# 1879615351/Go-RIO

Hardware: AMD Instinct MI355X
Metric: APD-GICP GN iters/sec on 16k-pt scans + GP-preint windows/sec (higher is better)
Workload: dtype f32 search / f64 accumulate; 1 GPU; C4: 64 scan pairs 16384x16384 + 64 GP windows 1 s @ 200 Hz per GPU, k-NN covariances + 20 fixed GN iterations per pair; pairs_per_gpu=64, target_points=16384, optimizer=GN (convergence test disabled), search=pruned, parallelism=batch shard x1 (no collective)

## Files before the change

go-rio_amd/csrc/ugpm_api.hip:

```cpp
#include <hip/hip_runtime.h>

#include <algorithm>
#include <cstdlib>
#include <chrono>
#include <cstdio>
#include <cstring>
#include <limits>
#include <memory>
#include <string>
#include <atomic>
#include <vector>

#include "../../include/gorio_ugpm.h"
#include "dev_buffer.h"
#include "ugpm_kernels.hip"
#include "ugpm_lpm_out.hip"
#include "ugpm_chunks.h"
#include "ugpm_windows.h"

using namespace gorio;
using namespace gorio::windows;

namespace {

// ... 58 lines not shown
  PinnedBuf pin_out;
  DevBuf<double> lpm_ws;
  DevBuf<int> lpm_ints;
  DevBuf<ug::LpmOutWin> d_lpm_wins;
  struct StageEvents { hipEvent_t a, b; int stage; };
  std::vector<StageEvents> ev;

  void drop_stage_events() {
    for (auto& e : ev) { hipEventDestroy(e.a); hipEventDestroy(e.b); }
    ev.clear();
  }
  void reset() {
    if (device >= 0) hipSetDevice(device);
    for (size_t g = 1; g < groups.size(); ++g) destroy_stream_pair(groups[g]);
    for (Group& g : groups) { hipEventDestroy(g.ev_done); hipEventDestroy(g.ev_tab); }
    groups.clear();
    destroy_stream_pair(main);
    if (ev_up) hipEventDestroy(ev_up);
    ev_up = nullptr;
    drop_stage_events();
    ws.reset(); d_wins.reset(); d_ints.reset(); d_diag.reset(); pin_in.reset(); pin_out.reset(); lpm_ws.reset(); lpm_ints.reset(); d_lpm_wins.reset();
    wins_cap = 0;
    lm_budget[0] = lm_budget[1] = 0;
    device = -1;
  }
  ~Ctx() { reset(); }
};
thread_local Ctx g_ctx;

struct Stage {
  Ctx& c;
  hipStream_t stream;
  size_t slot = 0;
  bool on = false;
  Stage(Ctx& c_, int s, hipStream_t st = nullptr) : c(c_), stream(st ? st : c_.main.s) {
    hipEvent_t a = nullptr, b = nullptr;
    if (hipEventCreate(&a) != hipSuccess || hipEventCreate(&b) != hipSuccess) return;
    slot = c.ev.size();
    c.ev.push_back({a, b, s});
    hipEventRecord(a, stream);
    on = true;
  }
  ~Stage() {
    if (on) hipEventRecord(c.ev[slot].b, stream);
  }
};
struct StageEventsGuard {
  Ctx& c;
  ~StageEventsGuard() { c.drop_stage_events(); }
};

struct Run : Ctx::Group {
  int g0 = 0, nw = 0;
  const UgpmWin* wins = nullptr;
  bool active = true;
};

struct Batch {
  const gorio_ugpm_window* windows;
  int nw;
  std::vector<HostWin> hw;
  std::vector<UgpmWin> dw;
  std::vector<int> ints, flags, lpm_ints_h;
  std::vector<double> lpm_in;
  std::vector<ug::LpmOutWin> lw;
  std::vector<size_t> out_offs;
  std::vector<Run> runs;
  size_t total_doubles = 0, total_in = 0, total_out = 0;
  double* out_region = nullptr;
  int max_S = 0, max_G = 2, max_V = 2, max_infer = 0, n_lpm = 0;
  bool rerun = false;
  bool looks = false;
  bool enqueued_blind[2] = {false, false};
  std::vector<int> final_status;
  int first_error = 0;
  std::string first_error_msg;
  void note_error(int i, int code, const std::string& m) {
    if (first_error) return;
    first_error = code;
    first_error_msg = "window " + std::to_string(i) + ": " + m;
  }
};

int ensure_context(Ctx& c, int device) {
  int ndev = 0;
  if (hipGetDeviceCount(&ndev) != hipSuccess || ndev <= 0) return ufail(GORIO_UGPM_ERR_NO_DEVICE, "no usable HIP device (no CPU fallback exists)");
  if (device < 0 || device >= ndev) return ufail(GORIO_UGPM_ERR_INVALID, "bad device ordinal");
  if (c.device != device) c.reset();
  UHIP(hipSetDevice(device));
  if (c.device == device) return 0;
  if (int rc = make_stream_pair(c.main)) return rc;
  UHIP(hipFuncSetAttribute(reinterpret_cast<const void*>(&ug::corr_diag_kernel<kSolveKmaxSmall>), hipFuncAttributeMaxDynamicSharedMemorySize, 140 * 1024));
  UHIP(hipFuncSetAttribute(reinterpret_cast<const void*>(&ug::corr_diag_kernel<kSolveKmaxFull>), hipFuncAttributeMaxDynamicSharedMemorySize, 140 * 1024));
  UHIP(hipFuncSetAttribute(reinterpret_cast<const void*>(&ug::infer_kernel<kSolveKmaxSmall>), hipFuncAttributeMaxDynamicSharedMemorySize, 17 * (6 * 160 + 16) * 8));
  UHIP(hipFuncSetAttribute(reinterpret_cast<const void*>(&ug::infer_kernel<kSolveKmaxFull>), hipFuncAttributeMaxDynamicSharedMemorySize, 17 * (6 * 160 + 16) * 8) );
  const void* fns[] = {reinterpret_cast<const void*>(&ug::ata_kernel<4, 16, kAtaTilesCorr>), reinterpret_cast<const void*>(&ug::ata_kernel<8, 16, kAtaTilesCorr>),
                       reinterpret_cast<const void*>(&ug::ata_kernel<16, 8, kAtaTilesCorr>), reinterpret_cast<const void*>(&ug::ata_kernel<4, 16, kAtaTilesLm>),
                       reinterpret_cast<const void*>(&ug::ata_kernel<8, 16, kAtaTilesLm>)};
  for (const void* f : fns) UHIP(hipFuncSetAttribute(f, hipFuncAttributeMaxDynamicSharedMemorySize, 144 * 1024));
  c.device = device;
  return 0;
}

void plan_windows(Batch& b) {
  b.hw.resize(b.nw);
  int total_infer = 0;
  for (int i = 0; i < b.nw; ++i) {
    const gorio_ugpm_window& w = b.windows[i];
    HostWin& h = b.hw[i];
    total_infer += std::max(0, w.n_infer);
    b.max_infer = std::max(b.max_infer, w.n_infer);
    std::string err;
    if (plan_window(w, h, err) != 0) {
      b.note_error(i, h.status, err);
    } else if (h.is_lpm) {
      b.n_lpm++;
    } else {
      b.max_S = std::max(b.max_S, h.S);
      b.total_in += input_slot(w, h);
      b.total_doubles += h.ws_doubles;
    }
  }
  for (const HostWin& h : b.hw) {
    b.max_G = std::max(b.max_G, h.is_lpm ? 2 : h.G);
    b.max_V = std::max(b.max_V, h.is_lpm ? 2 : h.V);
  }
  b.total_out = (size_t)total_infer * 83;
  b.total_doubles += b.total_in + b.total_out + 64;
}

int reserve_workspace(Ctx& c, const Batch& b) {
  const size_t nw = b.nw;
  UHIP(c.ws.reserve(b.total_doubles));
  UHIP(reserve_group(c.wins_cap, nw, nw, c.d_wins, nw, c.d_ints, kWinInts * nw, c.d_diag, 4 * nw));
  UHIP(c.pin_in.reserve(sizeof(double) * b.total_in, sizeof(double) * (b.total_in + b.total_in / 4 + 64)));
  const size_t down = sizeof(double) * (b.total_out + 4 * nw) + sizeof(int) * kWinInts * nw;
  UHIP(c.pin_out.reserve(down, down + down / 4 + 64));
  return 0;
}

int stage_and_upload(Ctx& c, Batch& b) {
  b.dw.resize(b.nw);
  b.ints.assign(kWinInts * (size_t)b.nw, 0);
  b.out_offs.assign(b.nw, 0);
  double* const in_region = c.ws.get();
  b.out_region = in_region + b.total_in;
  double* base = b.out_region + (b.total_out + 31) / 32 * 32;
  double* const stage_in = static_cast<double*>(c.pin_in.get());
  size_t in_off = 0, out_off = 0;
  for (int i = 0; i < b.nw; ++i) {
    const gorio_ugpm_window& w = b.windows[i];
    const HostWin& h = b.hw[i];
    UgpmWin& u = b.dw[i];
    std::memset(&u, 0, sizeof(u));
    u.lmi = c.d_ints + kWinInts * (size_t)i;
    u.status = c.d_ints + kWinInts * (size_t)i + 16;
    b.ints[kWinInts * (size_t)i + 16] = h.status;
    u.n_infer = std::max(0, w.n_infer);
    b.out_offs[i] = out_off;
    u.out = b.out_region + out_off;
    out_off += (size_t)u.n_infer * 83;
    if (h.status != 0) continue;
    if (h.is_lpm) {
      b.ints[kWinInts * (size_t)i + 16] = 1;
      u.n_infer = 0;
      continue;
    }
    carve(w, h, u, base, in_region + in_off, u.out);
    u.G = h.G; u.V = h.V; u.S = h.S;
    u.correlate = w.correlate ? 1 : 0; u.overlap = w.overlap;
    u.state_freq = h.state_freq;
    copy_noise_and_priors(w, u);
    base += h.ws_doubles;
    double* s = stage_in + in_off;
    const size_t padded = input_slot(w, h);
    for (size_t k = padded - 4; k < padded; ++k) s[k] = 0.0;
    s = stage_samples(s, w, h.g0, h.G, h.v0, h.V);
    std::copy(h.state_t.begin(), h.state_t.end(), s);
    in_off += padded;
  }
  if (b.total_in) UHIP(hipMemcpyAsync(in_region, stage_in, sizeof(double) * b.total_in, hipMemcpyHostToDevice, c.main.s));
  UHIP(hipMemcpyAsync(c.d_wins, b.dw.data(), sizeof(UgpmWin) * b.nw, hipMemcpyHostToDevice, c.main.s));
// ... 13 lines not shown
    LpmHost& L = lh[widx.size()];
    build_lpm_timeline(b.windows[i], L);
    widx.push_back(i);
    max_T = std::max(max_T, (int)L.tl.size());
    ug::LpmOutWin dummy;
    const LpmSize sz = carve_lpm(b.windows[i], L.tl.size(), dummy, nullptr, nullptr, nullptr);
    in_dbl += sz.in;
    dbl += sz.scratch + 8;
    nint += sz.ints;
  }
  UHIP(c.lpm_ws.reserve(in_dbl + dbl));
  UHIP(c.lpm_ints.reserve(nint));
  UHIP(c.d_lpm_wins.reserve(b.n_lpm));
  b.lw.resize(widx.size());
  b.lpm_in.assign(in_dbl, 0.0);
  b.lpm_ints_h.assign(nint, 0);
  LpmSize at;
  for (size_t k = 0; k < widx.size(); ++k) {
    const int i = widx[k];
    const gorio_ugpm_window& w = b.windows[i];
    const LpmHost& L = lh[k];
    ug::LpmOutWin& u = b.lw[k];
    std::memset(&u, 0, sizeof(u));
    const LpmSize sz = carve_lpm(w, L.tl.size(), u, c.lpm_ws.get() + at.in, c.lpm_ws.get() + in_dbl + at.scratch, c.lpm_ints.get() + at.ints);
    std::copy(L.tl.begin(), L.tl.end(), stage_samples(b.lpm_in.data() + at.in, w, 0, w.n_gyr, 0, w.n_vel));
    stage_lpm_tables(b.lpm_ints_h.data() + at.ints, L);
    at.in += sz.in; at.scratch += sz.scratch; at.ints += sz.ints;
    u.G = w.n_gyr; u.V = w.n_vel; u.T = (int)L.tl.size(); u.n_infer = w.n_infer;
    u.start_index = L.start_index; u.dt_index = L.dt_index;
    copy_noise_and_priors(w, u);
    u.out = b.dw[i].out;
    u.status = c.d_ints + kWinInts * (size_t)i + 17;
  }
  UHIP(hipMemcpyAsync(c.lpm_ws, b.lpm_in.data(), sizeof(double) * in_dbl, hipMemcpyHostToDevice, c.main.s));
  UHIP(hipMemcpyAsync(c.lpm_ints, b.lpm_ints_h.data(), sizeof(int) * nint, hipMemcpyHostToDevice, c.main.s));
  UHIP(hipMemcpyAsync(c.d_lpm_wins, b.lw.data(), sizeof(ug::LpmOutWin) * b.lw.size(), hipMemcpyHostToDevice, c.main.s));
  const int nl = (int)b.lw.size();
  if (nl > 0) {
    Stage st(c, 0);
    ug::lpm_out_steps_kernel<<<dim3((max_T + 255) / 256, 5, nl), 256, 0, c.main.s>>>(c.d_lpm_wins);
    ug::lpm_out_scan_kernel<<<dim3(5, nl), 64, 0, c.main.s>>>(c.d_lpm_wins);
    ug::lpm_out_finish_kernel<<<nl, 256, 0, c.main.s>>>(c.d_lpm_wins);
    UHIP(hipGetLastError());
  }
  return 0;
}

int open_groups(Ctx& c, Batch& b) {
  int n_groups = 1;
  if (const char* e = std::getenv("GORIO_UGPM_GROUPS")) n_groups = std::atoi(e);
  n_groups = std::max(1, std::min(std::min(n_groups, 8), b.nw));
  while ((int)c.groups.size() < n_groups) {
    Ctx::Group g;
    if (c.groups.empty()) static_cast<StreamPair&>(g) = c.main;
    else if (int rc = make_stream_pair(g)) return rc;
    UHIP(hipEventCreateWithFlags(&g.ev_done, hipEventDisableTiming));
    UHIP(hipEventCreateWithFlags(&g.ev_tab, hipEventDisableTiming));
    c.groups.push_back(g);
  }
  if (!c.ev_up) UHIP(hipEventCreateWithFlags(&c.ev_up, hipEventDisableTiming));
  UHIP(hipEventRecord(c.ev_up, c.main.s));
  b.runs.resize(n_groups);
  for (int g = 0; g < n_groups; ++g) {
    Run& r = b.runs[g];
    static_cast<Ctx::Group&>(r) = c.groups[g];
    r.g0 = (int)((long)b.nw * g / n_groups);
    r.nw = (int)((long)b.nw * (g + 1) / n_groups) - r.g0;
    r.wins = c.d_wins + r.g0;
    if (g > 0) UHIP(hipStreamWaitEvent(r.s, c.ev_up, 0));
  }
  return 0;
}

void launch_ata(Ctx& c, int max_S, const Run& r, int which, int decide = 0) {
  hipStream_t sq = which == 2 ? r.s2 : r.s;
  Stage st_ata(c, which == 2 ? 6 : 5, sq);
  const int n = (which == 2 ? 6 : 3) * max_S;
  const int tpg = which == 2 ? kAtaTilesCorr : kAtaTilesLm;
  const int dense = (g_debug_path.load() & 1) ? 1 : 0;
  const int ng = ata_cut(n, which == 2 && !dense ? 3 * max_S : n, tpg).groups();
  const int npad = ((n + 15) / 32) * 32 + 16;
  const int grid = ((r.nw + 7) / 8) * ng * 8;
  auto lds = [&](int kc) { return sizeof(double) * 2 * kc * (npad + 1); };
  if (which == 2) {
    if (npad <= 256) ug::ata_kernel<4, 16, kAtaTilesCorr><<<grid, 512, lds(16), sq>>>(r.wins, which, r.nw, ng, decide, dense);
    else if (npad <= 512) ug::ata_kernel<8, 16, kAtaTilesCorr><<<grid, 512, lds(16), sq>>>(r.wins, which, r.nw, ng, decide, dense);
    else ug::ata_kernel<16, 8, kAtaTilesCorr><<<grid, 512, lds(8), sq>>>(r.wins, which, r.nw, ng, decide, dense);
  } else {
    if (npad <= 256) ug::ata_kernel<4, 16, kAtaTilesLm><<<grid, 512, lds(16), sq>>>(r.wins, which, r.nw, ng, decide, dense);
    else ug::ata_kernel<8, 16, kAtaTilesLm><<<grid, 512, lds(16), sq>>>(r.wins, which, r.nw, ng, decide, dense);
  }
}

SolverSizes batch_sizes(const Batch& b) { return solver_sizes(b.max_S, (g_debug_path.load() & 4) != 0); }

void launch_gram(const Run& r, const SolverSizes& z) {
  const dim3 grid(6, r.nw);
  if (z.gram_rows == kGramRowsSmall) ug::gram_kernel<kGramRowsSmall, kGramKmax><<<grid, 256, 0, r.s>>>(r.wins);
  else if (z.gram_rows == kGramRows) ug::gram_kernel<kGramRows, kGramKmax><<<grid, 256, 0, r.s>>>(r.wins);
  else ug::gram_kernel<kCholRowsFull, kSolveKmaxFull><<<grid, 256, 0, r.s>>>(r.wins);
}

void launch_lm_step(const Run& r, const SolverSizes& z, int problem) {
  const dim3 grid(r.nw, problem == 1 ? kVelBlocks : 1);
  if (z.lm_rows == kLmRowsSmall) ug::lm_step_kernel<kLmRowsSmall><<<grid, 512, 0, r.s>>>(r.wins);
  else ug::lm_step_kernel<kCholRowsFull><<<grid, 512, 0, r.s>>>(r.wins);
}

void launch_corr_diag(const Run& r, const SolverSizes& z, int max_S) {
  const dim3 grid((6 * max_S + 15) / 16, r.nw);
  const size_t lds = sizeof(double) * 17 * (6 * max_S + 16);
  if (z.solve_kmax == kSolveKmaxSmall) ug::corr_diag_kernel<kSolveKmaxSmall><<<grid, 256, lds, r.s2>>>(r.wins);
  else ug::corr_diag_kernel<kSolveKmaxFull><<<grid, 256, lds, r.s2>>>(r.wins);
}

void launch_infer(const Run& r, const SolverSizes& z, int max_S, int max_infer) {
  const dim3 grid(std::max(1, max_infer), r.nw);
  const size_t lds = sizeof(double) * 17 * (6 * max_S + 16);
  if (z.solve_kmax == kSolveKmaxSmall) ug::infer_kernel<kSolveKmaxSmall><<<grid, 256, lds, r.s>>>(r.wins);
  else ug::infer_kernel<kSolveKmaxFull><<<grid, 256, lds, r.s>>>(r.wins);
}

int enqueue_tables_and_correlation(Ctx& c, Batch& b) {
  const int max_S = b.max_S;
  const SolverSizes sizes = batch_sizes(b);
  for (const Run& r : b.runs) {
    {
      Stage st(c, 0, r.s);
      ug::lpm_rot_kernel<<<dim3(r.nw, 5), 320, 0, r.s>>>(r.wins);
      ug::lpm_init_kernel<<<r.nw, 320, 0, r.s>>>(r.wins);
    }
    {
      Stage st(c, 1, r.s);
      launch_gram(r, sizes);
      ug::cross_kernel<<<dim3(12, r.nw, (std::max(b.max_G, b.max_V) + ug::kCrossRows - 1) / ug::kCrossRows), 256, sizeof(double) * ug::kCrossRows * (((max_S + 31) / 32) * 32 + 4), r.s>>>(r.wins);
    }
    UHIP(hipEventRecord(r.ev_tab, r.s));
    UHIP(hipStreamWaitEvent(r.s2, r.ev_tab, 0));
    {
      Stage st(c, 2, r.s2);
      ug::corr_jac_kernel<<<dim3(ug::kCorrJacParts, r.nw), 256, 0, r.s2>>>(r.wins);
      UHIP(hipEventRecord(r.ev_jac, r.s2));
      launch_ata(c, max_S, r, 2);
      ug::corr_factor_kernel<<<r.nw, 512, 0, r.s2>>>(r.wins);
      launch_corr_diag(r, sizes, max_S);
    }
    UHIP(hipEventRecord(r.ev_corr, r.s2));
  }
  return 0;
}

int run_fit(Ctx& c, Batch& b, int problem) {
  const int max_S = b.max_S;
  const SolverSizes sizes = batch_sizes(b);
  std::vector<int>& flags = b.flags;
  const bool lmtrace = std::getenv("GORIO_UGPM_LMTRACE") != nullptr;
  const bool speculative = g_speculative_rot.load() != 0;
  std::vector<std::unique_ptr<Stage>> st_lm;
  for (Run& r : b.runs) {
    st_lm.emplace_back(new Stage(c, 3, r.s));
    if (problem == 0) ug::rot_eval_kernel<<<dim3(r.nw, kEvalSplit), 256, 0, r.s>>>(r.wins, 2);
    else ug::vel_eval_kernel<<<dim3(r.nw, kEvalSplit), 256, 0, r.s>>>(r.wins, 2);
    launch_ata(c, max_S, r, problem);
    r.active = true;
  }
  for (int it = 0; it <= 51; ++it) {
    bool any = false;
    for (Run& r : b.runs) {
      if (!r.active) continue;
      any = true;
      launch_lm_step(r, sizes, problem);
      if (problem == 0 && speculative) {
        ug::rot_eval_kernel<<<dim3(r.nw, kEvalSplit), 256, 0, r.s>>>(r.wins, 3);
        launch_ata(c, max_S, r, problem, 1);
// ... 339 lines not shown
```

go-rio_amd/csrc/ugpm_device.h:

```cpp
#pragma once
#include <stdint.h>

namespace gorio {

constexpr int kAtaTilesLm = 24, kAtaTilesCorr = 48;
constexpr int kWinInts = 48;
constexpr int kLmiNeed = 18;
constexpr int kStatusUnfinished = 2;
constexpr int kCholRowsFull = 384;
constexpr int kVelBlocks = 3;

#if defined(__HIPCC__)
#define GORIO_HD __host__ __device__
#else
#define GORIO_HD
#endif

struct AtaCut {
  int ntile, q_zero, ng_dense, ng_skip;
  GORIO_HD int groups() const { return ng_dense + ng_skip; }
  GORIO_HD bool skips(int grp) const { return grp >= ng_dense; }
  GORIO_HD int q_lo(int grp) const {
    return grp < ng_dense ? (int)((long)grp * q_zero / ng_dense) : q_zero + (int)((long)(grp - ng_dense) * (ntile - q_zero) / ng_skip);
  }
  GORIO_HD int q_hi(int grp) const { return grp + 1 == groups() ? ntile : q_lo(grp + 1); }
};
GORIO_HD inline AtaCut ata_cut(int n, int zero_col, int tpg) {
  const int T = (n + 15) / 16, tz = zero_col >= n ? T : (zero_col + 15) / 16;
  AtaCut c;
  c.ntile = T * (T + 1) / 2;
  c.q_zero = tz * (tz + 1) / 2;
  c.ng_dense = (c.q_zero + tpg - 1) / tpg;
  c.ng_skip = (c.ntile - c.q_zero + tpg - 1) / tpg;
  return c;
}

struct UgpmWin {
  const double* gyr_t;
  const double* gyr;
  const double* vel_t;
  const double* vel;
  const double* infer_t;
  double* state_t;
  int G, V, S, n_infer;
  int correlate, overlap;
  double start_t, state_freq, gyr_var, vel_var;
  double gyr_bias[3], vel_bias[3];
  double vel_bias_std, gyr_bias_std;
  double* Rq;
  double* Rstart;
  double* velr;
  double* dp;
  double* r0;
  double* r1;
  double* s_dr;
  double* s_vel;
  double* hyper;
  double* d_r_dt_local;
  double* d_r_dt_local_shift;
  double* delta_r_time;
  double* delta_r_bw;
  double* d_r_bw_local_shift;
  double* Kinv;
  double* KKinv;
  double* KintKinv;
  double* var;
  double* wgp;
  double* sstd;
  double* KsKinv;
  double* KsIntKinv;
  double* KgyrIntKinv;
  double* KvelKinv;
  double* Jrot;
  double* Jvel;
  double* res;
  double* res_new;
  double* JtJ;
  double* lhs;
  double* lmv;
  double* sample_tmp;
  double* sample_tmp_c;
  double* Jc;
  double* Ac;
  double* Linv;
  double* dsc;
  double* alpha;
  double* state_r;
  double* d_state_bw;
  double* d_d_r_dt;
  double* d_vel_bv;
  double* d_vel_bw;
  double* d_vel_dt;
  double* out;
  double* lmc;
  int* lmi;
  int* status;
};

}
```

go-rio_amd/csrc/ugpm_kernels.hip:

```cpp
#include <hip/hip_runtime.h>
#include <math.h>

#include "ugpm_device.h"

namespace gorio {
namespace ug {

__device__ __forceinline__ UgpmWin load_win(const UgpmWin* __restrict__ wins, int i) {
  UgpmWin w;
  __builtin_memcpy(&w, (const __attribute__((address_space(4))) void*)(wins + i), sizeof(UgpmWin));
  return w;
}


#ifndef GORIO_UGPM_XCD
#define GORIO_UGPM_XCD 1
#endif
struct WinPart {
  int win, part, z;
};
__device__ __forceinline__ WinPart xcd_win_part() {
  WinPart r{(int)blockIdx.y, (int)blockIdx.x, (int)blockIdx.z};
#if GORIO_UGPM_XCD
  if (gridDim.y >= 16u && (gridDim.y & 7u) == 0u) {
    const unsigned int inner = gridDim.x * gridDim.z;
    const unsigned int L = blockIdx.x + gridDim.x * (blockIdx.y + gridDim.y * blockIdx.z);
    const unsigned int slot = L >> 3, in = slot % inner;
    r.win = (int)((slot / inner) * 8u + (L & 7u));
    r.part = (int)(in % gridDim.x);
    r.z = (int)(in / gridDim.x);
  }
#endif
  return r;
}

constexpr double kDt = 0.01;
constexpr double kBw = 0.0001;
constexpr double kExpTol = 1e-14;
constexpr double kPi = 3.14159265358979323846;

struct V3 {
  double x, y, z;
};
struct M3 {
  double m[9];
};
__device__ __forceinline__ V3 v3(double x, double y, double z) { return V3{x, y, z}; }
__device__ __forceinline__ V3 operator+(V3 a, V3 b) { return V3{a.x + b.x, a.y + b.y, a.z + b.z}; }
__device__ __forceinline__ V3 operator-(V3 a, V3 b) { return V3{a.x - b.x, a.y - b.y, a.z - b.z}; }
__device__ __forceinline__ V3 operator*(double s, V3 a) { return V3{s * a.x, s * a.y, s * a.z}; }
__device__ __forceinline__ double vnorm(V3 a) { return sqrt(a.x * a.x + a.y * a.y + a.z * a.z); }
__device__ __forceinline__ V3 cross(V3 a, V3 b) { return V3{a.y * b.z - a.z * b.y, a.z * b.x - a.x * b.z, a.x * b.y - a.y * b.x}; }
__device__ __forceinline__ M3 eye3() { return M3{{1, 0, 0, 0, 1, 0, 0, 0, 1}}; }
__device__ __forceinline__ M3 mmul(const M3& a, const M3& b) {
  M3 r;
#pragma unroll
  for (int i = 0; i < 3; ++i)
#pragma unroll
    for (int j = 0; j < 3; ++j) r.m[i * 3 + j] = a.m[i * 3] * b.m[j] + a.m[i * 3 + 1] * b.m[3 + j] + a.m[i * 3 + 2] * b.m[6 + j];
  return r;
}
__device__ __forceinline__ M3 mtr(const M3& a) { return M3{{a.m[0], a.m[3], a.m[6], a.m[1], a.m[4], a.m[7], a.m[2], a.m[5], a.m[8]}}; }
__device__ __forceinline__ V3 mvec(const M3& a, V3 v) { return V3{a.m[0] * v.x + a.m[1] * v.y + a.m[2] * v.z, a.m[3] * v.x + a.m[4] * v.y + a.m[5] * v.z, a.m[6] * v.x + a.m[7] * v.y + a.m[8] * v.z}; }
__device__ __forceinline__ M3 skew(V3 v) { return M3{{0.0, -v.z, v.y, v.z, 0.0, -v.x, -v.y, v.x, 0.0}}; }
__device__ __forceinline__ void store3(double* p, V3 v) { p[0] = v.x; p[1] = v.y; p[2] = v.z; }
__device__ __forceinline__ V3 load3(const double* p) { return V3{p[0], p[1], p[2]}; }
__device__ __forceinline__ void storeM(double* p, const M3& a) {
#pragma unroll
  for (int i = 0; i < 9; ++i) p[i] = a.m[i];
}
__device__ __forceinline__ M3 loadM(const double* p) {
  M3 a;
#pragma unroll
  for (int i = 0; i < 9; ++i) a.m[i] = p[i];
  return a;
}

__device__ M3 expMap(V3 v) {
  const double n2 = v.x * v.x + v.y * v.y + v.z * v.z;
  const double ang = sqrt(n2);
  V3 a = v;
  if (n2 > 0.0) a = (1.0 / ang) * v;
  const double s = sin(ang), c = cos(ang);
  const V3 sa = s * a, ca = (1.0 - c) * a;
// ... 1471 lines not shown
        }
      }
      __syncthreads();
      for (int q = threadIdx.x; q < cnt; q += blockDim.x) {
        const int i = part + kCorrJacParts * (qb + q);
        const double dtm = w.gyr_t[i] - w.start_t;
        double D[3][6];
        jacobian_res(v3(sdot[q][3] + dtm * w.hyper[3], sdot[q][4] + dtm * w.hyper[7], sdot[q][5] + dtm * w.hyper[11]),
                     v3(sdot[q][0] + w.hyper[3], sdot[q][1] + w.hyper[7], sdot[q][2] + w.hyper[11]), D);
        double* st = w.sample_tmp_c + (size_t)i * 24;
        for (int a = 0; a < 3; ++a)
          for (int k = 0; k < 6; ++k) st[a * 6 + k] = D[a][k];
      }
      __syncthreads();
    }
  }
  __syncthreads();
  {
    const int nmine = (G - part + kCorrJacParts - 1) / kCorrJacParts;
    for (int rr = wave; rr < nmine * 3; rr += 4) {
      const int i = part + kCorrJacParts * (rr / 3), a = rr % 3;
      const double* st = w.sample_tmp_c + (size_t)i * 24;
      double* row = J + (size_t)(3 * i + a) * n;
      for (int c = 0; c < 3; ++c) {
        const double f0 = st[a * 6 + c], f1 = st[a * 6 + c + 3];
        const double* k0 = w.KsIntKinv + ((size_t)c * G + i) * S;
        const double* k1 = w.KsKinv + ((size_t)c * G + i) * S;
        for (int j = lane; j < S; j += 64) row[c * S + j] = f0 * k0[j] + f1 * k1[j];
      }
    }
  }
  __syncthreads();
  {
    const int nmine = (V - part + kCorrJacParts - 1) / kCorrJacParts;
    for (int qb = 0; qb < nmine; qb += 256) {
      const int cnt = min(256, nmine - qb);
      for (int q = wave; q < cnt; q += 4) {
        const int i = part + kCorrJacParts * (qb + q);
        double d[6];
        wave_row_dots6(w.KgyrIntKinv + (size_t)i * S, (size_t)V * S, w.s_dr, w.KvelKinv + (size_t)i * S, (size_t)V * S, w.s_vel, S, d);
        if (lane == 0) {
#pragma unroll
          for (int q2 = 0; q2 < 6; ++q2) sdot[q][q2] = d[q2];
        }
      }
      __syncthreads();
      for (int q = threadIdx.x; q < cnt; q += blockDim.x) {
        const int i = part + kCorrJacParts * (qb + q);
        const double dtm = w.vel_t[i] - w.start_t;
        const V3 rv = v3(sdot[q][0] + dtm * w.hyper[3], sdot[q][1] + dtm * w.hyper[7], sdot[q][2] + dtm * w.hyper[11]);
        const M3 RT = expMap(v3(-rv.x, -rv.y, -rv.z));
        const V3 t = mvec(RT, v3(sdot[q][3] + w.hyper[15], sdot[q][4] + w.hyper[19], sdot[q][5] + w.hyper[23]));
        const M3 dres = mmul(skew(t), Jr(rv));
        double* st = w.sample_tmp_c + (size_t)i * 24;
        storeM(st, dres);
        storeM(st + 9, RT);
      }
      __syncthreads();
    }
  }
  __syncthreads();
  {
    const int nmine = (V - part + kCorrJacParts - 1) / kCorrJacParts;
    for (int rr = wave; rr < nmine * 3; rr += 4) {
      const int i = part + kCorrJacParts * (rr / 3), a = rr % 3;
      const double* st = w.sample_tmp_c + (size_t)i * 24;
      double* row = J + (size_t)(3 * G + 3 * i + a) * n;
      for (int c = 0; c < 3; ++c) {
        const double f0 = wgt * st[a * 3 + c], f1 = wgt * st[9 + a * 3 + c];
        const double* k0 = w.KgyrIntKinv + ((size_t)c * V + i) * S;
        const double* k1 = w.KvelKinv + ((size_t)c * V + i) * S;
        for (int j = lane; j < S; j += 64) {
          row[c * S + j] = f0 * k0[j];
          row[(3 + c) * S + j] = f1 * k1[j];
        }
      }
    }
  }
}


__device__ __forceinline__ int ata_npad(int n) { return ((n + 15) / 32) * 32 + 16; }

template <int CMAX, int KC, int TPG>
__global__ __launch_bounds__(512) void ata_kernel(const UgpmWin* __restrict__ wins, int which, int n_windows, int groups_max, int decide, int dense) {
  const int L = blockIdx.x;
  const int xcd = L & 7, slot = L >> 3;
#ifdef GORIO_ATA_NO_XCD
  const int win = (slot * 8 + xcd) / groups_max, grp = (slot * 8 + xcd) % groups_max;
#else
  const bool long_first = which == 2 && !dense;
  const int nrow = (n_windows + 7) / 8;
  const int win = (long_first ? slot % nrow : slot / groups_max) * 8 + xcd, grp = long_first ? slot / nrow : slot % groups_max;
#endif
  if (win >= n_windows) return;
  const UgpmWin w = load_win(wins, win);
  if (*w.status != 0) return;
  int m, n;
  const double* A;
  double* C;
  const double* r = nullptr;
  double* g = nullptr;
  int zrows = 0, zcol = 0;
  if (which == 2) {
    if (!w.correlate) return;
    m = 3 * w.G + 3 * w.V; n = 6 * w.S; A = w.Jc; C = w.Ac;
    zrows = 3 * w.G; zcol = 3 * w.S;
  } else {
    if (w.lmi[1]) return;
    n = 3 * w.S;
    m = which == 0 ? 3 * w.S + 3 * w.G : 3 * w.V + 3 * w.S;
    A = which == 0 ? w.Jrot : w.Jvel;
    C = w.JtJ; r = w.res; g = w.lmv;
    if (decide) {
      __shared__ double sred[8];
      if (lm_decide_block(w, m, n, grp == 0, sred) != 1) return;
      r = w.res_new;
      if (grp == 0)
        for (int k = threadIdx.x; k < m; k += blockDim.x) w.res[k] = r[k];
    } else if (!w.lmi[3]) {
      return;
    }
  }
  const AtaCut cut = ata_cut(n, zrows > 0 && !dense ? zcol : n, TPG);
  const int ng = cut.groups();
  if (grp >= ng) return;
  const int q_lo = cut.q_lo(grp), q_hi = cut.q_hi(grp);
  const int npad = ata_npad(n);
  const int nck = (m + KC - 1) / KC;
  const int c_lo = cut.skips(grp) ? zrows / KC : 0, c_hi = nck;
  extern __shared__ double ata_lds[];
  double* rl = ata_lds + (size_t)2 * KC * npad;
  const int tid = threadIdx.x, lane = tid & 63, wave = __builtin_amdgcn_readfirstlane(tid >> 6);
  const int lr = lane & 15, lk = lane >> 4;
  constexpr int NT = TPG / 8;
  int trofs[NT], tcofs[NT], qv[NT];
#pragma unroll
  for (int t = 0; t < NT; ++t) {
    const int q = min(q_lo + wave + 8 * t, q_hi - 1);
    int tr = (int)((sqrtf(8.0f * (float)q + 1.0f) - 1.0f) * 0.5f);
    while (tr * (tr + 1) / 2 > q) --tr;
    while ((tr + 1) * (tr + 2) / 2 <= q) ++tr;
    qv[t] = __builtin_amdgcn_readfirstlane(q);
    trofs[t] = __builtin_amdgcn_readfirstlane(tr) * 16;
    tcofs[t] = __builtin_amdgcn_readfirstlane(q - tr * (tr + 1) / 2) * 16;
  }
  const int nt = max(0, min(NT, (q_hi - q_lo - wave + 7) / 8));
  f64x4 acc[NT];
#pragma unroll
  for (int t = 0; t < NT; ++t) acc[t] = f64x4{0.0, 0.0, 0.0, 0.0};
  double gacc = 0.0;
  const int gj0 = (int)((long)grp * n / ng), gj1 = (int)((long)(grp + 1) * n / ng);
  const int gcolw = ((gj1 - gj0 + 63) / 64) * 64;
  const int gparts = gcolw <= 64 ? 8 : (gcolw <= 128 ? 4 : (gcolw <= 256 ? 2 : 1));
  const int gpart = (int)threadIdx.x / gcolw, gj = gj0 + (int)threadIdx.x % gcolw;
  const bool gcol = g != nullptr && gpart < gparts && gj < gj1;
  constexpr int RMAX = KC / 8;
  double pre[RMAX][CMAX];
  double rpre = 0.0;
  auto fetch = [&](int ck) {
#pragma unroll
    for (int rr = 0; rr < RMAX; ++rr) {
      const int k = ck * KC + wave + 8 * rr;
      const int ncol = k < zrows ? zcol : n;
#pragma unroll
      for (int cc = 0; cc < CMAX; ++cc) {
        const int col = lane + 64 * cc;
        pre[rr][cc] = (k < m && col < ncol) ? A[(size_t)k * n + col] : 0.0;
      }
    }
    if (r != nullptr && tid < KC) rpre = (ck * KC + tid < m) ? r[ck * KC + tid] : 0.0;
  };
  auto stash = [&](int buf) {
    double* dst = ata_lds + (size_t)buf * KC * npad;
#pragma unroll
    for (int rr = 0; rr < RMAX; ++rr) {
      const int row = wave + 8 * rr;
#pragma unroll
      for (int cc = 0; cc < CMAX; ++cc) {
        const int col = lane + 64 * cc;
        if (col < npad) dst[row * npad + col] = pre[rr][cc];
      }
    }
    if (tid < KC) rl[buf * KC + tid] = rpre;
  };
  CHOL_T_INIT;
  if (c_lo < c_hi) {
    fetch(c_lo);
    stash(0);
  }
  __syncthreads();
  CHOL_T(0);
  for (int ck = c_lo; ck < c_hi; ++ck) {
    const int buf = (ck - c_lo) & 1;
    if (ck + 1 < c_hi) fetch(ck + 1);
    const double* src = ata_lds + (size_t)buf * KC * npad;
#pragma unroll
    for (int kk = 0; kk < KC; kk += 4) {
      const double* rowp = src + (kk + lk) * npad + lr;
      double av[NT], bv[NT];
#pragma unroll
      for (int t = 0; t < NT; ++t) {
        av[t] = rowp[trofs[t]];
        bv[t] = rowp[tcofs[t]];
      }
#pragma unroll
      for (int t = 0; t < NT; ++t) acc[t] = __builtin_amdgcn_mfma_f64_16x16x4f64(av[t], bv[t], acc[t], 0, 0, 0);
    }
    CHOL_T(1);
    if (gcol) {
      for (int kk = gpart; kk < KC; kk += gparts) gacc += src[kk * npad + gj] * rl[buf * KC + kk];
    }
    CHOL_T(2);
    if (ck + 1 < c_hi) stash(buf ^ 1);
    CHOL_T(3);
    __syncthreads();
    CHOL_T(4);
  }
  {
#pragma unroll
    for (int t = 0; t < NT; ++t) {
      if (t < nt) {
#pragma unroll
        for (int rg = 0; rg < 4; ++rg) {
          const int i = trofs[t] + lk + 4 * rg, j = tcofs[t] + lr;
          if (i < n && j < n) {
            C[(size_t)i * n + j] = acc[t][rg];
            C[(size_t)j * n + i] = acc[t][rg];
          }
        }
      }
    }
    if (g != nullptr) {
      __syncthreads();
      if (gpart < gparts) ata_lds[gpart * gcolw + (int)threadIdx.x % gcolw] = gcol ? gacc : 0.0;
      __syncthreads();
      if (tid < gj1 - gj0) {
        double v = 0.0;
        for (int q = 0; q < gparts; ++q) v += ata_lds[q * gcolw + tid];
        g[gj0 + tid] = v;
      }
    }
  }
  CHOL_T(7);
}

__global__ __launch_bounds__(256) void lm_relinearize_linear_kernel(const UgpmWin* __restrict__ wins) {
  const UgpmWin w = load_win(wins, blockIdx.x);
  if (*w.status != 0 || w.lmi[1]) return;
  const int n = 3 * w.S, m = 3 * w.V + 3 * w.S;
  const int j0 = blockIdx.y * 64;
  if (j0 >= n) return;
  __shared__ double sred[8];
  if (lm_decide_block(w, m, n, blockIdx.y == 0, sred) != 1) return;
  const double* J = w.Jvel;
  const double* rn = w.res_new;
  __shared__ double sg[4][64];
  if (blockIdx.y == 0)
    for (int k = threadIdx.x; k < m; k += blockDim.x) w.res[k] = rn[k];
  const int slice = threadIdx.x >> 6, lane = threadIdx.x & 63;
  const int j = j0 + lane;
  double acc[4] = {0.0, 0.0, 0.0, 0.0};
  if (j < n) {
    int k = slice;
    for (; k + 12 < m; k += 16) {
#pragma unroll
      for (int u = 0; u < 4; ++u) acc[u] += J[(size_t)(k + 4 * u) * n + j] * rn[k + 4 * u];
    }
    for (; k < m; k += 4) acc[0] += J[(size_t)k * n + j] * rn[k];
  }
  sg[slice][lane] = (acc[0] + acc[1]) + (acc[2] + acc[3]);
  __syncthreads();
  if (slice == 0 && j < n) w.lmv[j] = (sg[0][lane] + sg[1][lane]) + (sg[2][lane] + sg[3][lane]);
}


__device__ void lm_begin_block(const UgpmWin& w, int problem) {
  const int n = 3 * w.S;
  const double* src = problem == 0 ? w.s_dr : w.s_vel;
  for (int j = threadIdx.x; j < n; j += blockDim.x) w.lmv[5 * (size_t)n + j] = src[j];
  if (threadIdx.x == 0) {
    for (int q = 0; q < 16; ++q) w.lmi[q] = 0;
    w.lmi[3] = 1;
    w.lmi[7] = problem;
    w.lmi[8] = 1;
    w.lmc[2] = 1e4;
    w.lmc[3] = 2.0;
  }
}

template <int ROWS>
__global__ __launch_bounds__(512) void lm_step_kernel(const UgpmWin* __restrict__ wins) {
  const UgpmWin w = load_win(wins, blockIdx.x);
  if (*w.status != 0 || w.lmi[1]) return;
  const int n = 3 * w.S;
  const int problem = w.lmi[7];
  const int m = problem == 0 ? 3 * w.S + 3 * w.G : 3 * w.V + 3 * w.S;
  const int nblk = (int)gridDim.y, blk = (int)blockIdx.y;
  const int j0 = (int)((long)n * blk / nblk), j1 = (int)((long)n * (blk + 1) / nblk), ns = j1 - j0;
  double* g = w.lmv;
  double* scale = w.lmv + (size_t)n;
  double* diag = w.lmv + 2 * (size_t)n;
  double* step = w.lmv + 3 * (size_t)n;
  double* delta = w.lmv + 4 * (size_t)n;
  double* x = w.lmv + 5 * (size_t)n;
// ... 407 lines not shown
```

go-rio_amd/ugpm.py:

```python
import ctypes as C

import numpy as np

from .apd import GorioError, load_library

LPM, UGPM = 0, 1
REC = 83

UGPM_SYMBOLS = ["gorio_ugpm_default_window", "gorio_ugpm_preint_batch", "gorio_ugpm_last_error", "gorio_ugpm_get_stage_times", "gorio_ugpm_debug_set_schedule",
                "gorio_ugpm_debug_set_path",                 "gorio_ugpm_combine_preints"]


class UgpmWindow(C.Structure):

    _fields_ = [
        ("gyr_t", C.c_void_p), ("gyr", C.c_void_p), ("n_gyr", C.c_int),
        ("vel_t", C.c_void_p), ("vel", C.c_void_p), ("n_vel", C.c_int),
        ("gyr_var", C.c_double), ("vel_var", C.c_double), ("start_t", C.c_double),
        ("infer_t", C.c_void_p), ("n_infer", C.c_int), ("type", C.c_int),
        ("min_freq", C.c_double), ("quantum", C.c_double), ("state_freq", C.c_double),
        ("correlate", C.c_int), ("overlap", C.c_int),
        ("gyr_bias", C.c_double * 3), ("vel_bias", C.c_double * 3),
        ("vel_bias_std", C.c_double), ("gyr_bias_std", C.c_double),
        ("group_sizes", C.c_void_p), ("n_groups", C.c_int),
# ... 30 lines not shown
        self.counts = []
        for i, w in enumerate(windows):
            lib.gorio_ugpm_default_window(C.byref(self.arr[i]))
            gt = np.ascontiguousarray(w["gyr_t"], np.float64)
            g = np.ascontiguousarray(w["gyr"], np.float64)
            vt = np.ascontiguousarray(w["vel_t"], np.float64)
            v = np.ascontiguousarray(w["vel"], np.float64)
            q = np.ascontiguousarray([w["end_t"]] if infer_t is None else infer_t[i], np.float64)
            self.keep += [gt, g, vt, v, q]
            a = self.arr[i]
            a.gyr_t, a.gyr, a.n_gyr = _dp(gt), _dp(g), len(gt)
            a.vel_t, a.vel, a.n_vel = _dp(vt), _dp(v), len(vt)
            a.gyr_var, a.vel_var, a.start_t = w["gyr_var"], w["vel_var"], w["start_t"]
            a.infer_t, a.n_infer = _dp(q), len(q)
            a.type, a.min_freq, a.state_freq = int(type), min_freq, state_freq
            a.quantum = float(quantum[i]) if np.ndim(quantum) > 0 else float(quantum)
            a.correlate, a.overlap = int(bool(correlate)), int(overlap)
            for k in range(3):
                a.gyr_bias[k] = 0.0 if gyr_bias is None else float(gyr_bias[k])
                a.vel_bias[k] = 0.0 if vel_bias is None else float(vel_bias[k])
            a.vel_bias_std, a.gyr_bias_std = vel_bias_std, gyr_bias_std
            if groups is not None and groups[i] is not None:
                gs = np.ascontiguousarray(groups[i], np.int32)
                assert int(gs.sum()) == len(q)
                self.keep.append(gs)
                a.group_sizes, a.n_groups = gs.__array_interface__["data"][0], len(gs)
            self.counts.append(len(q))
        self.out = np.zeros((sum(self.counts), REC))
        self.diag = (UgpmDiag * n)()

    def run(self):
        lib = load_library()
        rc = lib.gorio_ugpm_preint_batch(self.arr, self.n, C.c_void_p(_dp(self.out)), self.diag, self.device)
        if rc < 0:
            msg = lib.gorio_ugpm_last_error()
            raise GorioError(rc, msg.decode() if msg else "")
        return self.out

    def results(self):
        res, k = [], 0
        for cnt in self.counts:
            res.append([unpack(self.out[k + j]) for j in range(cnt)])
            k += cnt
        return res

    def diagnostics(self):
        return [dict(nb_state=d.nb_state, nb_gyr=d.nb_gyr, nb_vel=d.nb_vel, iters_rot=d.iters_rot, iters_vel=d.iters_vel, status=d.status,
                     cost_rot=d.cost_rot, cost_vel=d.cost_vel, state_freq=d.state_freq) for d in self.diag]


def ugpm_preint_batch(windows, device=0, infer_t=None, type=UGPM, state_freq=50.0, correlate=True, overlap=8, quantum=-1.0, min_freq=500.0,
                      gyr_bias=None, vel_bias=None, vel_bias_std=0.0, gyr_bias_std=0.0, return_diag=False, groups=None):
    b = UgpmBatch(windows, device=device, infer_t=infer_t, type=type, state_freq=state_freq, correlate=correlate, overlap=overlap, quantum=quantum,
                  min_freq=min_freq, gyr_bias=gyr_bias, vel_bias=vel_bias, vel_bias_std=vel_bias_std, gyr_bias_std=gyr_bias_std, groups=groups)
    b.run()
    if return_diag:
        return b.results(), b.diagnostics()
    return b.results()


def pack(m):
    return np.concatenate([np.asarray(m["delta_R"], np.float64).ravel(), np.asarray(m["delta_p"], np.float64), [m["dt"], m["dt_sq_half"]],
                           np.asarray(m["cov"], np.float64).ravel(), np.asarray(m["d_delta_R_d_bw"], np.float64).ravel(), np.asarray(m["d_delta_R_d_t"], np.float64),
                           np.asarray(m["d_delta_p_d_bw"], np.float64).ravel(), np.asarray(m["d_delta_p_d_bv"], np.float64).ravel(), np.asarray(m["d_delta_p_d_t"], np.float64)])


def ugpm_combine_preints(prev, cur):
    lib = load_library()
    a, b, out = np.ascontiguousarray(pack(prev)), np.ascontiguousarray(pack(cur)), np.zeros(REC)
    lib.gorio_ugpm_combine_preints.argtypes = [C.c_void_p, C.c_void_p, C.c_void_p]
    rc = lib.gorio_ugpm_combine_preints(C.c_void_p(_dp(a)), C.c_void_p(_dp(b)), C.c_void_p(_dp(out)))
    if rc < 0:
        raise GorioError(rc, lib.gorio_ugpm_last_error().decode())
    return unpack(out)


def ugpm_debug_set_schedule(speculative_rot=True):
    lib = load_library()
    lib.gorio_ugpm_debug_set_schedule.argtypes = [C.c_int]
    lib.gorio_ugpm_debug_set_schedule.restype = None
    lib.gorio_ugpm_debug_set_schedule(1 if speculative_rot else 0)


def ugpm_debug_set_path(dense_ata=False, draining_looks=False, full_capacity=False):
    lib = load_library()
    lib.gorio_ugpm_debug_set_path.argtypes = [C.c_int]
    lib.gorio_ugpm_debug_set_path.restype = None
    lib.gorio_ugpm_debug_set_path((1 if dense_ata else 0) | (2 if draining_looks else 0) | (4 if full_capacity else 0))


def ugpm_stage_times():
    lib = load_library()
    s = (C.c_double * 8)()
    c = (C.c_int * 8)()
    lib.gorio_ugpm_get_stage_times(s, c)
    return list(s), list(c)


class PreintOption:

    def __init__(self, min_freq=500.0, type=UGPM, quantum=-1.0, state_freq=50.0, correlate=True):
        self.min_freq, self.type, self.quantum, self.state_freq, self.correlate = min_freq, type, quantum, state_freq, correlate


class PreintPrior:

    def __init__(self, vel_bias=(0.0, 0.0, 0.0), gyr_bias=(0.0, 0.0, 0.0)):
        self.vel_bias, self.gyr_bias = list(vel_bias), list(gyr_bias)


class VelPreintegration:

    def __init__(self, imu_data, start_t, infer_t, opt=None, prior=None, rot_only=False, overlap=8, device=0):
        opt = opt or PreintOption()
        prior = prior or PreintPrior()
        if np.isscalar(infer_t):
            self._kind, groups = "single", [[float(infer_t)]]
        elif len(infer_t) and np.isscalar(infer_t[0]):
            self._kind, groups = "vec", [list(map(float, infer_t))]
        else:
            self._kind, groups = "vecvec", [list(map(float, g)) for g in infer_t]
        flat = [t for g in groups for t in g]
        win = dict(imu_data)
        win["start_t"] = start_t
        self._args = dict(device=device, infer_t=[flat], type=opt.type, state_freq=opt.state_freq, correlate=opt.correlate, overlap=overlap,
                          quantum=opt.quantum, min_freq=opt.min_freq, gyr_bias=prior.gyr_bias, vel_bias=prior.vel_bias,
                          groups=[[len(g) for g in groups]])
        self._win = win
        self._groups = groups
        self._prior = prior
        self._cache = {}

    def _compute(self, vel_bias_std, gyr_bias_std):
        key = (vel_bias_std, gyr_bias_std)
        if key not in self._cache:
            flat = ugpm_preint_batch([self._win], vel_bias_std=vel_bias_std, gyr_bias_std=gyr_bias_std, **self._args)[0]
            out, k = [], 0
            for g in self._groups:
                out.append(flat[k:k + len(g)])
                k += len(g)
            self._cache[key] = out
        return self._cache[key]

    def get(self, *idx, vel_bias_std=0.3, gyr_bias_std=0.03):
        pre = self._compute(vel_bias_std, gyr_bias_std)
        if len(idx) == 2:
            i, j = idx
        elif len(idx) == 1:
            if self._kind != "vec":
                raise IndexError("VelPreintegration::get: The type of query does not math the type of constructor")
            i, j = 0, idx[0]
        else:
            if self._kind != "single":
                raise IndexError("VelPreintegration::get: The type of query does not math the type of constructor")
            i, j = 0, 0
        if not (0 <= i < len(pre) and 0 <= j < len(pre[i])):
            raise IndexError("VelPreintegration::get: Trying to get precomputed preintegrated measurements (wrong index query?)")
        return pre[i][j]

    def getPrior(self):
        return self._prior
```

Measured before the change: 178,900 linearisations/s.

## Assign consecutive triangle tiles per wave in LM AᵀA to share row loads

For the LM-problem AᵀA kernel, each wave now owns a contiguous run of lower-triangle tiles instead of a stride-8 set. Consecutive tiles span at most two tile rows, so the A-operand can be reused from one row load plus the diagonal tile's B-operand, which cuts LDS reads per MFMA k-step. The old strided mapping stays available through a debug flag. The cost is more complex per-wave bookkeeping and a possibly different load balance across waves.

```diff
diff --git a/go-rio_amd/csrc/ugpm_api.hip b/go-rio_amd/csrc/ugpm_api.hip
--- a/go-rio_amd/csrc/ugpm_api.hip
+++ b/go-rio_amd/csrc/ugpm_api.hip
@@ -164,6 +164,14 @@
   }
 };
 
+using AtaFn = void (*)(const UgpmWin*, int, int, int, int, int);
+constexpr AtaFn kAtaCorr4 = &ug::ata_kernel<4, 16, kAtaTilesCorr, false>, kAtaCorr8 = &ug::ata_kernel<8, 16, kAtaTilesCorr, false>,
+                kAtaCorr16 = &ug::ata_kernel<16, 8, kAtaTilesCorr, false>;
+template <bool ROWMAP>
+constexpr AtaFn kAtaLm4 = &ug::ata_kernel<4, 16, kAtaTilesLm, ROWMAP>;
+template <bool ROWMAP>
+constexpr AtaFn kAtaLm8 = &ug::ata_kernel<8, 16, kAtaTilesLm, ROWMAP>;
+
 int ensure_context(Ctx& c, int device) {
   int ndev = 0;
   if (hipGetDeviceCount(&ndev) != hipSuccess || ndev <= 0) return ufail(GORIO_UGPM_ERR_NO_DEVICE, "no usable HIP device (no CPU fallback exists)");
@@ -176,10 +184,8 @@
   UHIP(hipFuncSetAttribute(reinterpret_cast<const void*>(&ug::corr_diag_kernel<kSolveKmaxFull>), hipFuncAttributeMaxDynamicSharedMemorySize, 140 * 1024));
   UHIP(hipFuncSetAttribute(reinterpret_cast<const void*>(&ug::infer_kernel<kSolveKmaxSmall>), hipFuncAttributeMaxDynamicSharedMemorySize, 17 * (6 * 160 + 16) * 8));
   UHIP(hipFuncSetAttribute(reinterpret_cast<const void*>(&ug::infer_kernel<kSolveKmaxFull>), hipFuncAttributeMaxDynamicSharedMemorySize, 17 * (6 * 160 + 16) * 8) );
-  const void* fns[] = {reinterpret_cast<const void*>(&ug::ata_kernel<4, 16, kAtaTilesCorr>), reinterpret_cast<const void*>(&ug::ata_kernel<8, 16, kAtaTilesCorr>),
-                       reinterpret_cast<const void*>(&ug::ata_kernel<16, 8, kAtaTilesCorr>), reinterpret_cast<const void*>(&ug::ata_kernel<4, 16, kAtaTilesLm>),
-                       reinterpret_cast<const void*>(&ug::ata_kernel<8, 16, kAtaTilesLm>)};
-  for (const void* f : fns) UHIP(hipFuncSetAttribute(f, hipFuncAttributeMaxDynamicSharedMemorySize, 144 * 1024));
+  for (AtaFn f : {kAtaCorr4, kAtaCorr8, kAtaCorr16, kAtaLm4<true>, kAtaLm4<false>, kAtaLm8<true>, kAtaLm8<false>})
+    UHIP(hipFuncSetAttribute(reinterpret_cast<const void*>(f), hipFuncAttributeMaxDynamicSharedMemorySize, 144 * 1024));
   c.device = device;
   return 0;
 }
@@ -359,14 +365,12 @@
   const int npad = ((n + 15) / 32) * 32 + 16;
   const int grid = ((r.nw + 7) / 8) * ng * 8;
   auto lds = [&](int kc) { return sizeof(double) * 2 * kc * (npad + 1); };
-  if (which == 2) {
-    if (npad <= 256) ug::ata_kernel<4, 16, kAtaTilesCorr><<<grid, 512, lds(16), sq>>>(r.wins, which, r.nw, ng, decide, dense);
-    else if (npad <= 512) ug::ata_kernel<8, 16, kAtaTilesCorr><<<grid, 512, lds(16), sq>>>(r.wins, which, r.nw, ng, decide, dense);
-    else ug::ata_kernel<16, 8, kAtaTilesCorr><<<grid, 512, lds(8), sq>>>(r.wins, which, r.nw, ng, decide, dense);
-  } else {
-    if (npad <= 256) ug::ata_kernel<4, 16, kAtaTilesLm><<<grid, 512, lds(16), sq>>>(r.wins, which, r.nw, ng, decide, dense);
-    else ug::ata_kernel<8, 16, kAtaTilesLm><<<grid, 512, lds(16), sq>>>(r.wins, which, r.nw, ng, decide, dense);
-  }
+  const bool rowmap = (g_debug_path.load() & 8) == 0;
+  AtaFn fn;
+  if (which == 2) fn = npad <= 256 ? kAtaCorr4 : (npad <= 512 ? kAtaCorr8 : kAtaCorr16);
+  else if (npad <= 256) fn = rowmap ? kAtaLm4<true> : kAtaLm4<false>;
+  else fn = rowmap ? kAtaLm8<true> : kAtaLm8<false>;
+  fn<<<grid, 512, lds(fn == kAtaCorr16 ? 8 : 16), sq>>>(r.wins, which, r.nw, ng, decide, dense);
 }
 
 SolverSizes batch_sizes(const Batch& b) { return solver_sizes(b.max_S, (g_debug_path.load() & 4) != 0); }
diff --git a/go-rio_amd/csrc/ugpm_device.h b/go-rio_amd/csrc/ugpm_device.h
--- a/go-rio_amd/csrc/ugpm_device.h
+++ b/go-rio_amd/csrc/ugpm_device.h
@@ -1,4 +1,5 @@
 #pragma once
+#include <math.h>
 #include <stdint.h>
 
 namespace gorio {
@@ -33,6 +34,54 @@
   c.ng_dense = (c.q_zero + tpg - 1) / tpg;
   c.ng_skip = (c.ntile - c.q_zero + tpg - 1) / tpg;
   return c;
+}
+
+constexpr int kAtaWaveTilesMax = 6, kAtaWaveRowsMax = 3;
+struct AtaWaveTiles {
+  int nrows;
+  int row[kAtaWaveRowsMax];
+  int diag[kAtaWaveRowsMax];
+  int slot[kAtaWaveTilesMax];
+  int col[kAtaWaveTilesMax];
+  int stored;
+};
+GORIO_HD inline int ata_tile_row(int q) {
+  int tr = (int)((sqrtf(8.0f * (float)q + 1.0f) - 1.0f) * 0.5f);
+  while (tr * (tr + 1) / 2 > q) --tr;
+  while ((tr + 1) * (tr + 2) / 2 <= q) ++tr;
+  return tr;
+}
+GORIO_HD inline AtaWaveTiles ata_wave_tiles(int q_lo, int q_hi, int wave, int nt) {
+  AtaWaveTiles m;
+  m.nrows = 0;
+  m.stored = 0;
+  for (int r = 0; r < kAtaWaveRowsMax; ++r) m.row[r] = m.diag[r] = 0;
+  for (int t = 0; t < kAtaWaveTilesMax; ++t) m.slot[t] = m.col[t] = 0;
+  int last = -1;
+#if defined(__HIP_DEVICE_COMPILE__)
+#pragma unroll
+#endif
+  for (int t = 0; t < kAtaWaveTilesMax; ++t) {
+    if (t >= nt) continue;
+    const int own = q_lo + wave * nt + t;
+    const int q = own < q_hi - 1 ? own : q_hi - 1;
+    const int tr = ata_tile_row(q);
+    if (tr != last) {
+#if defined(__HIP_DEVICE_COMPILE__)
+#pragma unroll
+#endif
+      for (int r = 0; r < kAtaWaveRowsMax; ++r) {
+        if (r == m.nrows) m.row[r] = tr;
+        if (r + 1 == m.nrows) m.diag[r] = t - 1;
+      }
+      ++m.nrows;
+      last = tr;
+    }
+    m.slot[t] = m.nrows - 1;
+    m.col[t] = q - tr * (tr + 1) / 2;
+    if (own < q_hi) m.stored |= 1 << t;
+  }
+  return m;
 }
 
 struct UgpmWin {
diff --git a/go-rio_amd/csrc/ugpm_kernels.hip b/go-rio_amd/csrc/ugpm_kernels.hip
--- a/go-rio_amd/csrc/ugpm_kernels.hip
+++ b/go-rio_amd/csrc/ugpm_kernels.hip
@@ -1,5 +1,6 @@
 #include <hip/hip_runtime.h>
 #include <math.h>
+#include <type_traits>
 
 #include "ugpm_device.h"
 
@@ -1637,7 +1638,7 @@
 
 __device__ __forceinline__ int ata_npad(int n) { return ((n + 15) / 32) * 32 + 16; }
 
-template <int CMAX, int KC, int TPG>
+template <int CMAX, int KC, int TPG, bool ROWMAP>
 __global__ __launch_bounds__(512) void ata_kernel(const UgpmWin* __restrict__ wins, int which, int n_windows, int groups_max, int decide, int dense) {
   const int L = blockIdx.x;
   const int xcd = L & 7, slot = L >> 3;
@@ -1689,18 +1690,34 @@
   const int tid = threadIdx.x, lane = tid & 63, wave = __builtin_amdgcn_readfirstlane(tid >> 6);
   const int lr = lane & 15, lk = lane >> 4;
   constexpr int NT = TPG / 8;
-  int trofs[NT], tcofs[NT], qv[NT];
-#pragma unroll
-  for (int t = 0; t < NT; ++t) {
-    const int q = min(q_lo + wave + 8 * t, q_hi - 1);
-    int tr = (int)((sqrtf(8.0f * (float)q + 1.0f) - 1.0f) * 0.5f);
-    while (tr * (tr + 1) / 2 > q) --tr;
-    while ((tr + 1) * (tr + 2) / 2 <= q) ++tr;
-    qv[t] = __builtin_amdgcn_readfirstlane(q);
-    trofs[t] = __builtin_amdgcn_readfirstlane(tr) * 16;
-    tcofs[t] = __builtin_amdgcn_readfirstlane(q - tr * (tr + 1) / 2) * 16;
-  }
-  const int nt = max(0, min(NT, (q_hi - q_lo - wave + 7) / 8));
+  int trofs[NT], tcofs[NT], tslot[NT];
+  int stored = 0, nrows = 0, rowl = 0, d0 = 0;
+  if constexpr (ROWMAP) {
+    static_assert(NT <= 3, "three consecutive tiles span at most two tile rows; the k-steps below know no third");
+    const AtaWaveTiles wt = ata_wave_tiles(q_lo, q_hi, wave, NT);
+#pragma unroll
+    for (int t = 0; t < NT; ++t) {
+      tslot[t] = __builtin_amdgcn_readfirstlane(wt.slot[t]);
+      trofs[t] = __builtin_amdgcn_readfirstlane(wt.slot[t] == 0 ? wt.row[0] : wt.row[1]) * 16;
+      tcofs[t] = __builtin_amdgcn_readfirstlane(wt.col[t]) * 16;
+    }
+    stored = __builtin_amdgcn_readfirstlane(wt.stored);
+    nrows = __builtin_amdgcn_readfirstlane(wt.nrows);
+    rowl = trofs[NT - 1];
+    d0 = __builtin_amdgcn_readfirstlane(wt.diag[0]);
+  } else {
+#pragma unroll
+    for (int t = 0; t < NT; ++t) {
+      const int own = q_lo + wave + 8 * t;
+      const int q = min(own, q_hi - 1);
+      const int tr = ata_tile_row(q);
+      tslot[t] = 0;
+      trofs[t] = __builtin_amdgcn_readfirstlane(tr) * 16;
+      tcofs[t] = __builtin_amdgcn_readfirstlane(q - tr * (tr + 1) / 2) * 16;
+      if (own < q_hi) stored |= 1 << t;
+    }
+    stored = __builtin_amdgcn_readfirstlane(stored);
+  }
   f64x4 acc[NT];
 #pragma unroll
   for (int t = 0; t < NT; ++t) acc[t] = f64x4{0.0, 0.0, 0.0, 0.0};
@@ -1746,21 +1763,42 @@
   }
   __syncthreads();
   CHOL_T(0);
+  auto ksteps = [&](auto nr, const double* src) {
+    constexpr int NR = decltype(nr)::value;
+#pragma unroll
+    for (int kk = 0; kk < KC; kk += 4) {
+      const double* rowp = src + (kk + lk) * npad + lr;
+      double av[NT], bv[NT];
+#pragma unroll
+      for (int t = 0; t < NT; ++t) bv[t] = rowp[tcofs[t]];
+      if constexpr (NR == 0) {
+#pragma unroll
+        for (int t = 0; t < NT; ++t) av[t] = rowp[trofs[t]];
+      } else {
+        const double rlast = rowp[rowl];
+        double r0 = bv[0];
+#pragma unroll
+        for (int t = 1; t + 1 < NT; ++t) r0 = (NR == 2 && d0 == t) ? bv[t] : r0;
+#pragma unroll
+        for (int t = 0; t < NT; ++t) {
+          if (NR == 1 || t == NT - 1) av[t] = rlast;
+          else if (t == 0) av[t] = r0;
+          else av[t] = tslot[t] == 0 ? r0 : rlast;
+        }
+      }
+#pragma unroll
+      for (int t = 0; t < NT; ++t) acc[t] = __builtin_amdgcn_mfma_f64_16x16x4f64(av[t], bv[t], acc[t], 0, 0, 0);
+    }
+  };
   for (int ck = c_lo; ck < c_hi; ++ck) {
     const int buf = (ck - c_lo) & 1;
     if (ck + 1 < c_hi) fetch(ck + 1);
     const double* src = ata_lds + (size_t)buf * KC * npad;
-#pragma unroll
-    for (int kk = 0; kk < KC; kk += 4) {
-      const double* rowp = src + (kk + lk) * npad + lr;
-      double av[NT], bv[NT];
-#pragma unroll
-      for (int t = 0; t < NT; ++t) {
-        av[t] = rowp[trofs[t]];
-        bv[t] = rowp[tcofs[t]];
-      }
-#pragma unroll
-      for (int t = 0; t < NT; ++t) acc[t] = __builtin_amdgcn_mfma_f64_16x16x4f64(av[t], bv[t], acc[t], 0, 0, 0);
+    if constexpr (!ROWMAP) {
+      ksteps(std::integral_constant<int, 0>{}, src);
+    } else {
+      if (nrows == 1) ksteps(std::integral_constant<int, 1>{}, src);
+      else ksteps(std::integral_constant<int, 2>{}, src);
     }
     CHOL_T(1);
     if (gcol) {
@@ -1775,7 +1813,7 @@
   {
 #pragma unroll
     for (int t = 0; t < NT; ++t) {
-      if (t < nt) {
+      if ((stored >> t) & 1) {
 #pragma unroll
         for (int rg = 0; rg < 4; ++rg) {
           const int i = trofs[t] + lk + 4 * rg, j = tcofs[t] + lr;
diff --git a/go-rio_amd/ugpm.py b/go-rio_amd/ugpm.py
--- a/go-rio_amd/ugpm.py
+++ b/go-rio_amd/ugpm.py
@@ -136,11 +136,11 @@
     lib.gorio_ugpm_debug_set_schedule(1 if speculative_rot else 0)
 
 
-def ugpm_debug_set_path(dense_ata=False, draining_looks=False, full_capacity=False):
+def ugpm_debug_set_path(dense_ata=False, draining_looks=False, full_capacity=False, strided_ata=False):
     lib = load_library()
     lib.gorio_ugpm_debug_set_path.argtypes = [C.c_int]
     lib.gorio_ugpm_debug_set_path.restype = None
-    lib.gorio_ugpm_debug_set_path((1 if dense_ata else 0) | (2 if draining_looks else 0) | (4 if full_capacity else 0))
+    lib.gorio_ugpm_debug_set_path((1 if dense_ata else 0) | (2 if draining_looks else 0) | (4 if full_capacity else 0) | (8 if strided_ata else 0))
 
 
 def ugpm_stage_times():
```

After: 186,200 linearisations/s, median of 4. +4.1%, better.
